# jianhao2016/AllSet

Measured on AMD Instinct MI355X. Metric: edges*d aggregated / sec (V->E->V layer fwd+bwd), higher is better.
Workload: dtype f32

## Files before the change

allset_amd/csrc/fused_fwd2.hip:

```cpp
#include <stdlib.h>

#include "common.h"
#include "mfma.h"

namespace allset {

constexpr int kF2Block = 768;
constexpr int kF2Rows = 32;
constexpr int kF2VWaves = 8;
constexpr int kF2Sets = 4;

#ifdef ALLSET_ABL5_NOBAR
#define ALLSET_TICK() ALLSET_TICK_NO_BARRIER()
#else
#define ALLSET_TICK() ALLSET_TICK_BARRIER()
#endif

template <bool HAS_LN, bool DROP_IN, bool DROP_OUT, bool D8, bool F16, int XM = 0, bool AUX = false>
__global__ __launch_bounds__(kF2Block) void fused_linear_fwd_roles_kernel(
    const float* __restrict__ x, int64_t ldx, const float* __restrict__ gamma, const float* __restrict__ beta, float eps,
    int relu_in, float p_in, uint64_t seed_in, const float* __restrict__ W, const float* __restrict__ bias, int relu_out,
    float p_out, uint64_t seed_out, float* __restrict__ y, int64_t ldy, float* __restrict__ stats, int64_t n,
    const uint64_t* __restrict__ seed_base, uint32_t* __restrict__ mask_out, int64_t xcb, int64_t ycb, float ln_inv,
    const float* __restrict__ colb = nullptr, float* __restrict__ uo = nullptr, int64_t lduo = 0,
// ... 139 lines not shown
        const float s = row16_sum(((t[0].x + t[0].y) + (t[0].z + t[0].w)) + ((t[1].x + t[1].y) + (t[1].z + t[1].w)));
        const float mean = s * inv_k;
        float q2 = 0.f;
#pragma unroll
        for (int hb = 0; hb < 2; ++hb) {
          t[hb].x -= mean; t[hb].y -= mean; t[hb].z -= mean; t[hb].w -= mean;
          q2 = fmaf(t[hb].x, t[hb].x, fmaf(t[hb].y, t[hb].y, fmaf(t[hb].z, t[hb].z, fmaf(t[hb].w, t[hb].w, q2))));
        }
        const float rstd = rsqrtf(row16_sum(q2) * inv_k + eps);
        if (live && c == 0) *reinterpret_cast<float2*>(stats + (stage * R + lr) * 2) = make_float2(mean, rstd);
#pragma unroll
        for (int hb = 0; hb < 2; ++hb) {
          t[hb].x = fmaf(t[hb].x * rstd, gam[hb].x, bet[hb].x); t[hb].y = fmaf(t[hb].y * rstd, gam[hb].y, bet[hb].y);
          t[hb].z = fmaf(t[hb].z * rstd, gam[hb].z, bet[hb].z); t[hb].w = fmaf(t[hb].w * rstd, gam[hb].w, bet[hb].w);
        }
      }
      if constexpr (XM == 1) {
        if (live) {
          char* ub = reinterpret_cast<char*>(uo + stage * R * lduo) + static_cast<uint32_t>(lr) * static_cast<uint32_t>(lduo) * 4u + 16u * c;
          *reinterpret_cast<float4*>(ub) = t[0];
          *reinterpret_cast<float4*>(ub + 256) = t[1];
        }
      }
      if constexpr (AUX) {
        float s4[4];
#pragma unroll
        for (int j = 0; j < 4; ++j) {
          const float4 w0 = *reinterpret_cast<const float4*>(&sAuxW[j * KD + 4 * c]), w1 = *reinterpret_cast<const float4*>(&sAuxW[j * KD + 64 + 4 * c]);
          s4[j] = row16_sum(fmaf(t[0].x, w0.x, fmaf(t[0].y, w0.y, fmaf(t[0].z, w0.z, t[0].w * w0.w))) +
                              fmaf(t[1].x, w1.x, fmaf(t[1].y, w1.y, fmaf(t[1].z, w1.z, t[1].w * w1.w))));
        }
        if (live && c == 0)
          *reinterpret_cast<float4*>(aux_out + (stage * R + lr) * 4) =
              make_float4(s4[0] + sAuxW[4 * KD], s4[1] + sAuxW[4 * KD + 1], s4[2] + sAuxW[4 * KD + 2], s4[3] + sAuxW[4 * KD + 3]);
      }
      float rsc = su1;
      if constexpr (ROWSC) {
        float amax = 0.f;
#pragma unroll
        for (int hb = 0; hb < 2; ++hb)
          amax = fmaxf(fmaxf(fmaxf(fabsf(t[hb].x), fabsf(t[hb].y)), fmaxf(fabsf(t[hb].z), fabsf(t[hb].w))), amax);
        amax = fmaxf(amax, dpp_row<0xB1>(amax)); amax = fmaxf(amax, dpp_row<0x4E>(amax));
        amax = fmaxf(amax, dpp_row<0x141>(amax)); amax = fmaxf(amax, dpp_row<0x140>(amax));
        const int e = min(max(static_cast<int>(__float_as_uint(amax * keep_in) >> 23), 20), 254);
        eC = eB; eB = eA; eA = e;
        rsc = __uint_as_float(static_cast<uint32_t>(254 + 13 - e) << 23);
      }
#pragma unroll
      for (int hb = 0; hb < 2; ++hb) {
        if constexpr (DROP_IN) {
          const float4 kp = keep4(seed_in, stage, hb, thr_in, keep_in);
          t[hb].x *= kp.x; t[hb].y *= kp.y; t[hb].z *= kp.z; t[hb].w *= kp.w;
        }
        if constexpr (ROWSC || XM == 1) { t[hb].x *= rsc; t[hb].y *= rsc; t[hb].z *= rsc; t[hb].w *= rsc; }
        const int wo = swizzle256(lr, 128 * hb + 8 * c);
        if constexpr (F16) {
          uint32_t h0, l0, h1, l1;
          split2_f16(t[hb].x, t[hb].y, h0, l0);
          split2_f16(t[hb].z, t[hb].w, h1, l1);
          *reinterpret_cast<uint2*>(img + 0 * PLANE + wo) = make_uint2(h0, h1);
          *reinterpret_cast<uint2*>(img + 1 * PLANE + wo) = make_uint2(l0, l1);
        } else {
          uint32_t h0, m0, l0, h1, m1, l1;
          split3_bf16(t[hb].x, t[hb].y, h0, m0, l0);
          split3_bf16(t[hb].z, t[hb].w, h1, m1, l1);
          *reinterpret_cast<uint2*>(img + 0 * PLANE + wo) = make_uint2(h0, h1);
          *reinterpret_cast<uint2*>(img + 1 * PLANE + wo) = make_uint2(m0, m1);
          *reinterpret_cast<uint2*>(img + 2 * PLANE + wo) = make_uint2(l0, l1);
        }
      }
      __builtin_amdgcn_sched_barrier(0);
      request_x(k + kF2Sets, xr);
      __builtin_amdgcn_sched_barrier(0);
    };
    auto E = [&](int64_t k, int erow) {
      const int64_t stage = stage_of(k);
      const int nrows = rows_left(stage);
      const bool live = lr < nrows;
      const float* ty = sY + (k & 1) * (R * SPY);
      char* yb = reinterpret_cast<char*>(y + stage * R * ldy);
      const uint32_t yo = static_cast<uint32_t>(lr) * static_cast<uint32_t>(ldy) * 4u + coy0;
      const float unsc = ROWSC ? __uint_as_float(static_cast<uint32_t>(erow - 13) << 23) : 1.f;
      float4 vv[2];
#pragma unroll
      for (int hb = 0; hb < 2; ++hb) {
        float4 v = *reinterpret_cast<const float4*>(&ty[lr * SPY + 64 * hb + 4 * c]);
        if constexpr (ROWSC) {
          v.x = fmaf(v.x, unsc, bia[hb].x); v.y = fmaf(v.y, unsc, bia[hb].y); v.z = fmaf(v.z, unsc, bia[hb].z); v.w = fmaf(v.w, unsc, bia[hb].w);
        } else {
          v.x += bia[hb].x; v.y += bia[hb].y; v.z += bia[hb].z; v.w += bia[hb].w;
        }
        if (relu_out) { v.x = fmaxf(v.x, 0.f); v.y = fmaxf(v.y, 0.f); v.z = fmaxf(v.z, 0.f); v.w = fmaxf(v.w, 0.f); }
        vv[hb] = v;
      }
      if constexpr (XM == 2) {
        float4 sv[2];
        float a1 = 0.f;
#pragma unroll
        for (int hb = 0; hb < 2; ++hb) {
          sv[hb] = make_float4(resR[hb].x + vv[hb].x, resR[hb].y + vv[hb].y, resR[hb].z + vv[hb].z, resR[hb].w + vv[hb].w);
          a1 += (sv[hb].x + sv[hb].y) + (sv[hb].z + sv[hb].w);
        }
        const float mean = row16_sum(a1) * (1.f / 128.f);
        float q2 = 0.f;
        float4 cv[2];
#pragma unroll
        for (int hb = 0; hb < 2; ++hb) {
          cv[hb] = make_float4(sv[hb].x - mean, sv[hb].y - mean, sv[hb].z - mean, sv[hb].w - mean);
          q2 = fmaf(cv[hb].x, cv[hb].x, fmaf(cv[hb].y, cv[hb].y, fmaf(cv[hb].z, cv[hb].z, fmaf(cv[hb].w, cv[hb].w, q2))));
        }
        const float rstd = rsqrtf(row16_sum(q2) * (1.f / 128.f) + eps);
        if (live) {
          if (c == 0) *reinterpret_cast<float2*>(stats + (stage * R + lr) * 2) = make_float2(mean, rstd);
          char* ub = reinterpret_cast<char*>(uo + stage * R * lduo) + static_cast<uint32_t>(lr) * static_cast<uint32_t>(lduo) * 4u + 16u * c;
          *reinterpret_cast<float4*>(ub) = sv[0];
          *reinterpret_cast<float4*>(ub + 256) = sv[1];
        }
#pragma unroll
        for (int hb = 0; hb < 2; ++hb) {
          float4 o = make_float4(fmaf(cv[hb].x * rstd, gam[hb].x, bet[hb].x), fmaf(cv[hb].y * rstd, gam[hb].y, bet[hb].y),
                                 fmaf(cv[hb].z * rstd, gam[hb].z, bet[hb].z), fmaf(cv[hb].w * rstd, gam[hb].w, bet[hb].w));
          if (relu_post) { o.x = fmaxf(o.x, 0.f); o.y = fmaxf(o.y, 0.f); o.z = fmaxf(o.z, 0.f); o.w = fmaxf(o.w, 0.f); }
          if constexpr (DROP_OUT) {
            const float4 kp = keep4(seed_out, stage, hb, thr_out, keep_out);
            o.x *= kp.x; o.y *= kp.y; o.z *= kp.z; o.w *= kp.w;
          }
          if (live) *reinterpret_cast<float4*>(yb + hb * dhy + yo) = o;
        }
      }
#pragma unroll
      for (int hb = 0; hb < 2; ++hb) {
        float4 v = vv[hb];
        if constexpr (DROP_OUT && XM != 2) {
          const float4 kp = keep4(seed_out, stage, hb, thr_out, keep_out);
          v.x *= kp.x; v.y *= kp.y; v.z *= kp.z; v.w *= kp.w;
        }
        if constexpr (XM == 3 || XM == 4) vv[hb] = v;
#ifdef ALLSET_ABL5_NOSTORE
        if (live && v.x == 123.456f)
#else
        if (live && XM != 2 && XM != 3 && XM != 4)
#endif
          *reinterpret_cast<float4*>(yb + hb * dhy + yo) = v;
        if (mask_out != nullptr) {
          const uint64_t b0 = __ballot(v.x > 0.f), b1 = __ballot(v.y > 0.f), b2 = __ballot(v.z > 0.f), b3 = __ballot(v.w > 0.f);
          const int sh = 8 * (lane0 & 7);
          const uint32_t word = static_cast<uint32_t>((b0 >> sh) & 0xffu) | (static_cast<uint32_t>((b1 >> sh) & 0xffu) << 8) |
                                (static_cast<uint32_t>((b2 >> sh) & 0xffu) << 16) | (static_cast<uint32_t>((b3 >> sh) & 0xffu) << 24);
          if (lane0 < 8 && 16 * (wave >> 2) < nrows)
            mask_out[((stage * (R / 16) + (wave >> 2)) * (ND / 64) + hb) * 32 + (wave & 3) * 8 + lane0] = word;
        }
      }
      if constexpr (XM == 3 || XM == 4) {
        uint32_t u[2][4], own[2], oth[2];
        const uint32_t sh = 4u * (c & 7);
#pragma unroll
        for (int hb = 0; hb < 2; ++hb) {
          u[hb][0] = __float_as_uint(vv[hb].x); u[hb][1] = __float_as_uint(vv[hb].y);
          u[hb][2] = __float_as_uint(vv[hb].z); u[hb][3] = __float_as_uint(vv[hb].w);
          const uint32_t nib = (u[hb][0] != 0u ? 1u : 0u) | (u[hb][1] != 0u ? 2u : 0u) | (u[hb][2] != 0u ? 4u : 0u) | (u[hb][3] != 0u ? 8u : 0u);
          float mw = __uint_as_float(nib << sh);
          mw = __uint_as_float(__float_as_uint(mw) | __float_as_uint(dpp_row<0xB1>(mw)));
          mw = __uint_as_float(__float_as_uint(mw) | __float_as_uint(dpp_row<0x4E>(mw)));
          mw = __uint_as_float(__float_as_uint(mw) | __float_as_uint(dpp_row<0x141>(mw)));
          own[hb] = __float_as_uint(mw);
          oth[hb] = __float_as_uint(dpp_row<0x140>(mw));
        }
        const bool hi = c >= 8;
        const uint32_t below = (1u << sh) - 1u;
        const int cnt0 = __popc(own[0]) + __popc(oth[0]);
        const int kocc = cnt0 + __popc(own[1]) + __popc(oth[1]);
        int pos[2];
        pos[0] = 4 + (hi ? __popc(oth[0]) : 0) + __popc(own[0] & below);
        pos[1] = 4 + cnt0 + (hi ? __popc(oth[1]) : 0) + __popc(own[1] & below);
        uint32_t* im = reinterpret_cast<uint32_t*>(sY + (k & 1) * (R * SPY) + lr * SPY);
        __builtin_amdgcn_fence(__ATOMIC_SEQ_CST, "wavefront");
        __builtin_amdgcn_wave_barrier();
        if constexpr (XM == 4) {
          *reinterpret_cast<uint4*>(im + 4 * c) = make_uint4(0u, 0u, 0u, (128u + c) * 0x010101u | (static_cast<uint32_t>(kocc) << 24));
          uint8_t* imb = reinterpret_cast<uint8_t*>(im);
#pragma unroll
          for (int hb = 0; hb < 2; ++hb) {
            int j = pos[hb] - 4;
#pragma unroll
            for (int i = 0; i < 4; ++i) {
              const bool put = u[hb][i] != 0u && j < kCellCap;
              const int cl = 16 * (j & 15), sl = j >> 4;
              *reinterpret_cast<uint32_t*>(imb + (put ? cl + 4 * sl : 4 * (SPY - 1))) = u[hb][i];
              imb[put ? cl + 12 + sl : 4 * (SPY - 1)] = static_cast<uint8_t>(64 * hb + 4 * c + i);
              j += u[hb][i] != 0u ? 1 : 0;
            }
          }
        } else {
        *reinterpret_cast<uint4*>(im + 4 * c) = make_uint4(0u, 0u, 0u, 0u);
        *reinterpret_cast<uint4*>(im + (hi ? SPY - 4 : 0)) = make_uint4(own[0], oth[0], own[1], oth[1]);
#pragma unroll
        for (int hb = 0; hb < 2; ++hb)
#pragma unroll
          for (int i = 0; i < 4; ++i) {
            const bool occ = u[hb][i] != 0u;
            im[occ ? pos[hb] : SPY - 1] = u[hb][i];
            pos[hb] += occ ? 1 : 0;
          }
        }
        __builtin_amdgcn_fence(__ATOMIC_SEQ_CST, "wavefront");
        __builtin_amdgcn_wave_barrier();
        const uint4 o = *reinterpret_cast<const uint4*>(im + 4 * c);
        if (live) *reinterpret_cast<uint4*>(reinterpret_cast<uint32_t*>(uo) + (stage * R + lr) * kPackPitchDw + 4 * c) = o;
        if (live && kocc > (XM == 4 ? kCellCap : kPackCap)) {
          *reinterpret_cast<float4*>(yb + yo) = vv[0];
          *reinterpret_cast<float4*>(yb + 256 + yo) = vv[1];
        }
      }
      if constexpr (XM == 2) {
        __builtin_amdgcn_sched_barrier(0);
        request_res(k + 1);
        __builtin_amdgcn_sched_barrier(0);
      }
    };

    static_assert(kF2Sets == 4, "the trip below is written for four register sets");
#pragma unroll
    for (int q = 0; q < kF2Sets; ++q) request_x(q, xrS[q]);
    request_res(0);
    S0(0, xrS[0]);
    ALLSET_TICK();
    S0(1, xrS[1]);
    ALLSET_TICK();
#define ALLSET_F2_FULL_TICK(tt, set) do { ALLSET_MARK(3); S0((tt) + 1, xrS[set]); ALLSET_MARK(0); E((tt) - 1, eC); ALLSET_MARK(1); ALLSET_TICK(); ALLSET_MARK(2); } while (0)
    int64_t t = 1;
    for (; t + 3 < T; t += 4) {
      ALLSET_F2_FULL_TICK(t, 2);
      ALLSET_F2_FULL_TICK(t + 1, 3);
      ALLSET_F2_FULL_TICK(t + 2, 0);
      ALLSET_F2_FULL_TICK(t + 3, 1);
    }
    if (t < T) ALLSET_F2_FULL_TICK(t, 2);
    if (t + 1 < T) ALLSET_F2_FULL_TICK(t + 1, 3);
    if (t + 2 < T) ALLSET_F2_FULL_TICK(t + 2, 0);
#undef ALLSET_F2_FULL_TICK
    E(T - 1, eB);
  } else {
    const int m = wave - kF2VWaves;
    Frag wq[2][4][F16 ? 2 : 3];
    float inv_s = 1.f;
    if constexpr (F16) {
      const int nn = lane0 & 15, kg = lane0 >> 4;
      float4 wa[2][4], wb[2][4];
      float amax = 0.f;
#pragma unroll
      for (int ct = 0; ct < 2; ++ct)
#pragma unroll
        for (int tt = 0; tt < 4; ++tt) {
          const float4* wr = reinterpret_cast<const float4*>(W + (32 * m + 16 * ct + nn) * KD + 32 * kg + 8 * tt);
          wa[ct][tt] = wr[0]; wb[ct][tt] = wr[1];
          amax = fmaxf(fmaxf(fmaxf(fabsf(wa[ct][tt].x), fabsf(wa[ct][tt].y)), fmaxf(fabsf(wa[ct][tt].z), fabsf(wa[ct][tt].w))), amax);
          amax = fmaxf(fmaxf(fmaxf(fabsf(wb[ct][tt].x), fabsf(wb[ct][tt].y)), fmaxf(fabsf(wb[ct][tt].z), fabsf(wb[ct][tt].w))), amax);
        }
#pragma unroll
      for (int off = 1; off < 64; off <<= 1) amax = fmaxf(amax, __shfl_xor(amax, off));
      const int ew = __builtin_amdgcn_readfirstlane(min(max(static_cast<int>(__float_as_uint(amax) >> 23), 20), 254));
      const float sw = __uint_as_float(static_cast<uint32_t>(254 + 13 - ew) << 23);
      const int X = ew - 140 - Su, X1 = X >> 1, X2 = X - X1;
      inv_s = __uint_as_float(static_cast<uint32_t>(127 + X1) << 23) * __uint_as_float(static_cast<uint32_t>(127 + X2) << 23);
#pragma unroll
      for (int ct = 0; ct < 2; ++ct)
#pragma unroll
        for (int tt = 0; tt < 4; ++tt) {
          const float4 a = wa[ct][tt], b = wb[ct][tt];
          uint32_t ph[4], pl[4];
          split2_f16(a.x * sw, a.y * sw, ph[0], pl[0]);
          split2_f16(a.z * sw, a.w * sw, ph[1], pl[1]);
          split2_f16(b.x * sw, b.y * sw, ph[2], pl[2]);
          split2_f16(b.z * sw, b.w * sw, ph[3], pl[3]);
          wq[ct][tt][0].u = make_uint4(ph[0], ph[1], ph[2], ph[3]);
          wq[ct][tt][1].u = make_uint4(pl[0], pl[1], pl[2], pl[3]);
        }
    } else {
      const int nn = lane0 & 15, kg = lane0 >> 4;
#pragma unroll
      for (int ct = 0; ct < 2; ++ct)
#pragma unroll
        for (int tt = 0; tt < 4; ++tt) {
          const float4* wr = reinterpret_cast<const float4*>(W + (32 * m + 16 * ct + nn) * KD + 32 * kg + 8 * tt);
          const float4 a = wr[0], b = wr[1];
          uint32_t ph[4], pm[4], pl[4];
          split3_bf16(a.x, a.y, ph[0], pm[0], pl[0]);
          split3_bf16(a.z, a.w, ph[1], pm[1], pl[1]);
          split3_bf16(b.x, b.y, ph[2], pm[2], pl[2]);
          split3_bf16(b.z, b.w, ph[3], pm[3], pl[3]);
          wq[ct][tt][0].u = make_uint4(ph[0], ph[1], ph[2], ph[3]);
          wq[ct][tt][1].u = make_uint4(pm[0], pm[1], pm[2], pm[3]);
          wq[ct][tt][2].u = make_uint4(pl[0], pl[1], pl[2], pl[3]);
        }
    }
    auto S1 = [&](int64_t k) {
      ALLSET_FRESH_LANE(lane);
      const int ri = lane & 15, kg = lane >> 4;
      const uint8_t* img = sX + (k & 1) * IMG;
      float* ty = sY + (k & 1) * (R * SPY);
      constexpr int NP = F16 ? 2 : 3;
      auto load_a = [&](Frag (&f0)[3], Frag (&f1)[3], int tt) {
        const int o0 = swizzle256(ri, 64 * kg + 16 * tt), o1 = swizzle256(16 + ri, 64 * kg + 16 * tt);
#pragma unroll
        for (int pl = 0; pl < NP; ++pl) {
          f0[pl].u = *reinterpret_cast<const uint4*>(img + pl * PLANE + o0);
          f1[pl].u = *reinterpret_cast<const uint4*>(img + pl * PLANE + o1);
        }
      };
      Frag fa0[2][3], fa1[2][3];
      f32x4 acc[2][2];
#pragma unroll
      for (int a = 0; a < 2; ++a)
#pragma unroll
        for (int b = 0; b < 2; ++b) acc[a][b] = f32x4{0.f, 0.f, 0.f, 0.f};
      load_a(fa0[0], fa1[0], 0);
#pragma unroll
      for (int tt = 0; tt < 4; ++tt) {
        if (tt + 1 < 4) load_a(fa0[(tt + 1) & 1], fa1[(tt + 1) & 1], tt + 1);
        const Frag (&a0)[3] = fa0[tt & 1];
        const Frag (&a1)[3] = fa1[tt & 1];
        constexpr int PA_[6] = {2, 0, 1, 1, 0, 0}, PB_[6] = {0, 2, 1, 0, 1, 0};
#ifdef ALLSET_ABL5_NOMFMA
        acc[0][0][0] += __builtin_bit_cast(float, a0[0].u.x ^ a0[1].u.y ^ a0[2].u.z); acc[1][0][0] += __builtin_bit_cast(float, a1[0].u.x ^ a1[1].u.y ^ a1[2].u.z);
        for (int pr = 0; pr < 0; ++pr) {
#else
#pragma unroll
        for (int pr = 0; pr < (F16 ? 0 : 6); ++pr) {
#endif
          if constexpr (!F16) {
            acc[0][0] = __builtin_amdgcn_mfma_f32_16x16x32_bf16(a0[PA_[pr]].v, wq[0][tt][PB_[pr]].v, acc[0][0], 0, 0, 0);
            acc[1][0] = __builtin_amdgcn_mfma_f32_16x16x32_bf16(a1[PA_[pr]].v, wq[0][tt][PB_[pr]].v, acc[1][0], 0, 0, 0);
            acc[0][1] = __builtin_amdgcn_mfma_f32_16x16x32_bf16(a0[PA_[pr]].v, wq[1][tt][PB_[pr]].v, acc[0][1], 0, 0, 0);
            acc[1][1] = __builtin_amdgcn_mfma_f32_16x16x32_bf16(a1[PA_[pr]].v, wq[1][tt][PB_[pr]].v, acc[1][1], 0, 0, 0);
          }
        }
#ifndef ALLSET_ABL5_NOMFMA
        if constexpr (F16) {
          constexpr int QA_[3] = {1, 0, 0}, QB_[3] = {0, 1, 0};
#pragma unroll
          for (int pr = 0; pr < 3; ++pr) {
            acc[0][0] = __builtin_amdgcn_mfma_f32_16x16x32_f16(a0[QA_[pr]].h, wq[0][tt][QB_[pr]].h, acc[0][0], 0, 0, 0);
            acc[1][0] = __builtin_amdgcn_mfma_f32_16x16x32_f16(a1[QA_[pr]].h, wq[0][tt][QB_[pr]].h, acc[1][0], 0, 0, 0);
            acc[0][1] = __builtin_amdgcn_mfma_f32_16x16x32_f16(a0[QA_[pr]].h, wq[1][tt][QB_[pr]].h, acc[0][1], 0, 0, 0);
            acc[1][1] = __builtin_amdgcn_mfma_f32_16x16x32_f16(a1[QA_[pr]].h, wq[1][tt][QB_[pr]].h, acc[1][1], 0, 0, 0);
          }
        }
#endif
        __builtin_amdgcn_sched_barrier(0);
      }
#pragma unroll
      for (int rt = 0; rt < 2; ++rt)
#pragma unroll
        for (int ct = 0; ct < 2; ++ct)
#pragma unroll
          for (int r = 0; r < 4; ++r) ty[(16 * rt + 4 * kg + r) * SPY + 32 * m + 16 * ct + ri] = F16 ? acc[rt][ct][r] * inv_s : acc[rt][ct][r];
    };
    ALLSET_TICK();
    for (int64_t k = 0; k < T; ++k) {
      ALLSET_MARK(3);
// ... 221 lines not shown
```

allset_amd/dense.py:

```python
from __future__ import annotations

import contextlib
import os
from ctypes import byref, c_int64
from typing import Optional, Tuple

import torch
from torch.autograd.function import once_differentiable

from . import _lib, _memo
from ._lib import check, ptr, require_device, stream_of, on_device
from .ops import _ld, _rowmajor, _timed

Tensor = torch.Tensor


class _SeedSource:
    base: Optional[Tensor] = None
    salt: int = 0


_SEED_SCRATCH = torch.empty((), dtype=torch.int64)


# ... 918 lines not shown
        _check_f32(x)
        x = x.contiguous()
        y = torch.empty_like(x)
        seed, base = _seed_for(p)
        n = x.numel()
        with on_device(dev), _timed("relu_dropout_fwd", dev, 2 * n * 4):
            check(_lib.load().allset_relu_dropout_fwd(ptr(x), p, seed, ptr(y), n, ptr(base),
                                                      stream_of(dev)), "allset_relu_dropout_fwd")
        ctx.save_for_backward(y)
        ctx.p = float(p)
        return y

    @staticmethod
    @once_differentiable
    def backward(ctx, gy):
        (y,) = ctx.saved_tensors
        dev = y.device
        gy = gy.contiguous()
        gx = torch.empty_like(y)
        n = y.numel()
        with on_device(dev), _timed("relu_dropout_bwd", dev, 3 * n * 4):
            check(_lib.load().allset_relu_dropout_bwd(ptr(gy), ptr(y), ctx.p, ptr(gx), n, stream_of(dev)),
                  "allset_relu_dropout_bwd")
        return gx, None


class _Linear(torch.autograd.Function):

    @staticmethod
    def forward(ctx, x, weight, bias):
        ctx.save_for_backward(x, weight)
        ctx.has_bias = bias is not None
        ctx.params = (weight, bias)
        return torch.nn.functional.linear(x, weight, bias)

    @staticmethod
    @once_differentiable
    def backward(ctx, gy):
        x, weight = ctx.saved_tensors
        gy = gy.contiguous()
        gx = gw = gb = None
        need_w, need_b = ctx.needs_input_grad[1], ctx.has_bias and ctx.needs_input_grad[2]
        if need_w and linear_narrow_supported(gy, x, weight):
            defer = ctx.params if (not ctx.has_bias or need_b) else None
            gx, gw, gb = linear_narrow_bwd(gy, x, weight, ctx.needs_input_grad[0], defer_to=defer)
            return gx, gw, gb if need_b else None
        if ctx.needs_input_grad[0]:
            gx = gy @ weight
        if need_w or need_b:
            if wgrad_supported(gy, x):
                gw, gb = wgrad(gy, x, want_bias=need_b)
            elif (gy.is_cuda and gy.dtype == x.dtype and gy.dtype in (torch.float32, torch.bfloat16) and x.dim() == 2
                  and gy.shape[0] >= 8192):
                gw, gb = wgrad_padded(gy, x, want_bias=need_b)
            else:
                gw = gy.t() @ x
                gb = gy.sum(dim=0) if need_b else None
        return gx, gw, gb


class _FusedNormLinear(torch.autograd.Function):

    @staticmethod
    def forward(ctx, x, gamma, beta, weight, bias, eps, relu_in, p_in, relu_out, p_out, in_cb=0, out_cb=0):
        seed_in = _draw_seed() if p_in > 0.0 else 0
        seed_out = _draw_seed() if p_out > 0.0 else 0
        base = _seed_base() if (p_in > 0.0 or p_out > 0.0) else None
        keep_y = relu_out or p_out > 0.0
        words = activation_mask_words(x.shape[0], weight.shape[0]) if (keep_y and any(ctx.needs_input_grad)) else 0
        mask = torch.empty(words, dtype=torch.int32, device=x.device) if words > 0 else None
        if in_cb or out_cb:
            n_rows = x.shape[0] // (weight.shape[1] // in_cb) if in_cb else x.shape[0]
            words = activation_mask_words(n_rows, weight.shape[0]) if (keep_y and any(ctx.needs_input_grad)) else 0
            mask = torch.empty(words, dtype=torch.int32, device=x.device) if words > 0 else None
            y, stats = fused_linear_fwd_blocked(x, in_cb, weight, bias, gamma, beta, eps, relu_in, p_in, seed_in, relu_out, p_out,
                                                seed_out, base, mask, out_cb)
        else:
            y, stats = fused_linear_fwd(x, weight, bias, gamma, beta, eps, relu_in, p_in, seed_in, relu_out, p_out, seed_out,
                                        base, mask)
        ctx.save_for_backward(x, stats, gamma, beta, weight, y if (keep_y and mask is None) else None, mask)
        ctx.cfg = (bool(relu_in), float(p_in), seed_in, float(p_out), bias is not None, base)
        ctx.layout = (int(in_cb), int(out_cb))
        ctx.params = (gamma, beta, weight, bias)
        return y

    @staticmethod
    @once_differentiable
    def backward(ctx, gy):
        x, stats, gamma, beta, weight, y, mask = ctx.saved_tensors
        relu_in, p_in, seed_in, p_out, has_bias, base = ctx.cfg
        if x.shape[0] == 0:
            z = lambda t, need: torch.zeros_like(t) if (t is not None and need) else None
            return (z(x, ctx.needs_input_grad[0]), z(gamma, ctx.needs_input_grad[1]), z(beta, ctx.needs_input_grad[2]),
                    z(weight, ctx.needs_input_grad[3]),
                    weight.new_zeros(weight.shape[0]) if (has_bias and ctx.needs_input_grad[4]) else None,
                    None, None, None, None, None, None, None)
        gy = gy.contiguous()
        gx = dg = db = gw = gb = None
        need_b = has_bias and ctx.needs_input_grad[4]
        in_cb, out_cb = ctx.layout
        if in_cb or out_cb:
            gx, dg, db, gw, gb = fused_linear_bwd_all_blocked(gy, out_cb, mask, p_out, weight, x, in_cb, stats, gamma, beta, relu_in,
                                                              p_in, seed_in, base, want_bias=need_b)
            return gx, dg, db, gw, gb, None, None, None, None, None, None, None
        if (ctx.needs_input_grad[0] and ctx.needs_input_grad[3] and y is None and x.shape[0] > 0 and
                (gamma is not None or one_pass_preferred(weight.shape[0], weight.shape[1])) and
                fused_linear_bwd_all_supported(weight.shape[0], weight.shape[1], gamma is not None, p_in > 0.0, relu_in,
                                               mask is not None)):
            need = ctx.needs_input_grad
            defer = ctx.params if (_Deferred.active and (gamma is None or (need[1] and need[2])) and (not has_bias or need[4])) else None
            gx, dg, db, gw, gb = fused_linear_bwd_all(gy, mask, p_out, weight, x, stats, gamma, beta, relu_in, p_in, seed_in,
                                                      base, want_bias=need_b, defer_to=defer)
            return gx, dg, db, gw, gb, None, None, None, None, None, None, None
        if ctx.needs_input_grad[3] or need_b:
            gw, gb = wgrad_fused(gy, y, p_out, x, stats, gamma, beta, relu_in, p_in, seed_in, want_bias=need_b,
                                 seed_base=base, mask=mask)
        if ctx.needs_input_grad[0] or (gamma is not None and (ctx.needs_input_grad[1] or ctx.needs_input_grad[2])):
            gx, dg, db = fused_linear_bwd(gy, y, p_out, weight, x, stats, gamma, relu_in, p_in, seed_in, base, mask,
                                          want_gx=ctx.needs_input_grad[0])
        return gx, dg, db, gw, gb, None, None, None, None, None, None, None


class PackedRows:

    __slots__ = ("packed", "_side", "format")

    def __init__(self, packed: Tensor, side: Tensor, format: str):
        from . import ops
        ops.packed_format_entry(format, "PackedRows")
        self.packed, self._side, self.format = packed, side, format

    @property
    def shape(self):
        return self._side.shape


class _FusedNormLinearPacked(torch.autograd.Function):

    @staticmethod
    def forward(ctx, x, gamma, beta, weight, bias, eps, relu_in, p_in, relu_out, p_out, fmt):
        from . import ops
        seed_in = _draw_seed()
        seed_out = _draw_seed()
        base = _seed_base()
        words = activation_mask_words(x.shape[0], weight.shape[0]) if any(ctx.needs_input_grad) else 0
        mask = torch.empty(words, dtype=torch.int32, device=x.device) if words > 0 else None
        packed, side, stats = ops.fused_linear_fwd_packed(x, weight, bias, gamma, beta, eps, relu_in, p_in, seed_in, relu_out, p_out, seed_out,
                                                          base, mask, _arith_for(0, weight.shape[1], weight.shape[0], True, 0), fmt=fmt)
        ctx.save_for_backward(x, stats, gamma, beta, weight, None, mask)
        ctx.cfg = (bool(relu_in), float(p_in), seed_in, float(p_out), bias is not None, base)
        ctx.layout = (0, 0)
        ctx.params = (gamma, beta, weight, bias)
        ctx.mark_non_differentiable(packed)
        return side, packed

    @staticmethod
    @once_differentiable
    def backward(ctx, gy, _g_packed=None):
        return _FusedNormLinear.backward(ctx, gy)[:10] + (None,)


def fused_norm_linear_packed_supported(x: Tensor, gamma: Optional[Tensor], weight: Tensor, p_in: float, relu_out: bool, p_out: float,
                                       format: str) -> bool:
    from . import ops
    N, K = weight.shape
    return (x.is_cuda and x.dtype == torch.float32 and x.dim() == 2 and x.shape[0] > 0 and gamma is not None and bool(relu_out)
            and ops.fused_linear_fwd_packed_supported(K, N, True, p_in, p_out, fmt=format))


def fused_norm_linear_packed(x: Tensor, gamma: Tensor, beta: Tensor, weight: Tensor, bias: Optional[Tensor], eps: float, relu_in: bool,
                             p_in: float, relu_out: bool, p_out: float, format: str) -> PackedRows:
    if not fused_norm_linear_packed_supported(x, gamma, weight, p_in, relu_out, p_out, format):
        raise _lib.AllSetHipError("fused_norm_linear_packed: built for a [128, 128] Linear behind a LayerNorm with relu_out and both "
                                  "dropouts active only (fused_norm_linear_packed_supported)")
    side, packed = _FusedNormLinearPacked.apply(x, gamma, beta, weight, bias, float(eps), bool(relu_in), float(p_in), bool(relu_out),
                                                float(p_out), format)
    return PackedRows(packed, side, format)


class _WideNormLinear(torch.autograd.Function):

    @staticmethod
    def forward(ctx, x, gamma, beta, weight, bias, eps, relu_in, p_in, relu_out, p_out, stats_in=None, emit=None):
        seed_in = _draw_seed() if p_in > 0.0 else 0
        seed_out = _draw_seed() if p_out > 0.0 else 0
        base = _seed_base() if (p_in > 0.0 or p_out > 0.0) else None
        stats = (stats_in if stats_in is not None else row_stats(x, relu_in, eps)) if gamma is not None else None
        stats_y = torch.empty((x.shape[0], 2), dtype=torch.float32, device=x.device) if emit is not None else None
        keep_y = relu_out or p_out > 0.0
        words = activation_mask_words(x.shape[0], weight.shape[0]) if (keep_y and x.shape[0] > 0) else 0
        mask = torch.empty(words, dtype=torch.int32, device=x.device) if words > 0 else None
        f16 = wide_f16(gamma is not None)
        planes, ctx.planes_t = (prefetched_planes(weight, False), prefetched_planes(weight, True)) if f16 else (None, None)
        y = gemm_x6(x, planes or gemm_x6_planes(weight, False, f16=f16), weight.shape[0], bias, relu_in=relu_in, stats=stats, gamma=gamma,
                    beta=beta, p_in=p_in, seed_in=seed_in, relu_out=relu_out, p_out=p_out, seed_out=seed_out, seed_base=base,
                    mask_out=mask, stats_out=stats_y, stats_eps=emit[0] if emit is not None else 1e-5,
                    stats_relu=bool(emit[1]) if emit is not None else False)
        ctx.save_for_backward(x, stats, gamma, beta, weight, y if (keep_y and mask is None) else None, mask)
        ctx.cfg = (bool(relu_in), float(p_in), seed_in, float(p_out), bias is not None, base)
        ctx.params = (gamma, beta, weight, bias)
        if emit is None:
            return y
        ctx.mark_non_differentiable(stats_y)
        return y, stats_y

    @staticmethod
    @once_differentiable
    def backward(ctx, gy, _g_stats=None):
        x, stats, gamma, beta, weight, y, mask = ctx.saved_tensors
        relu_in, p_in, seed_in, p_out, has_bias, base = ctx.cfg
        if x.shape[0] == 0:
            z = lambda t, need: torch.zeros_like(t) if (t is not None and need) else None
            return (z(x, ctx.needs_input_grad[0]), z(gamma, ctx.needs_input_grad[1]), z(beta, ctx.needs_input_grad[2]),
                    z(weight, ctx.needs_input_grad[3]),
                    weight.new_zeros(weight.shape[0]) if (has_bias and ctx.needs_input_grad[4]) else None,
                    None, None, None, None, None, None, None)
        gy = gy.contiguous()
        gx = dg = db = gw = gb = None
        need_b = has_bias and ctx.needs_input_grad[4]
        need = ctx.needs_input_grad
        p_g, p_bt, p_w, p_b = ctx.params
        dfr = _Deferred.active
        if ctx.needs_input_grad[3] or need_b:
            gw, gb = wgrad_fused(gy, y, p_out, x, stats, gamma, beta, relu_in, p_in, seed_in, want_bias=need_b, seed_base=base, mask=mask,
                                 defer_to=(p_w, p_b) if (dfr and need[3] and (not has_bias or need[4])) else None)
        need_x = ctx.needs_input_grad[0]
        if need_x or (gamma is not None and (ctx.needs_input_grad[1] or ctx.needs_input_grad[2])):
            planes_t = ctx.planes_t if (ctx.planes_t is not None and wide_f16()) else gemm_x6_planes(weight, True)
            if gamma is not None and weight.shape[1] <= 256:
                gx, dg, db = gemm_x6_lnb(gy, planes_t, x, stats, gamma, relu_in, p_in, seed_in, mask_y=y,
                                         p_mask=p_out, seed_base=base, mask_bits=mask,
                                         defer_to=(p_g, p_bt) if (dfr and need[1] and need[2]) else None)
                return gx, dg, db, gw, gb, None, None, None, None, None, None, None
            sgn = x if (gamma is None and relu_in and planes_t.f16 and x.stride(-1) == 1 and x.stride(0) % 4 == 0 and x.data_ptr() % 16 == 0
                        and _lib.load().allset_gemm_wide_sgn_supported(_lib.ARITH_FP16X3, weight.shape[1], weight.shape[0])) else None
            gu = gemm_x6(gy, planes_t, weight.shape[1], None, mask_y=y, p_mask=p_out, mask_bits=mask, sgn_x=sgn)
            if gamma is not None:
                gx, dg, db = ln_bwd(gu, x, stats, gamma, relu_in, p_in, seed_in, base, want_gx=need_x,
                                    defer_to=(p_g, p_bt) if (dfr and need[1] and need[2]) else None)
            elif relu_in and sgn is None:
                gx = torch.empty_like(x)
                with torch.cuda.device(x.device), _timed("relu_dropout_bwd", x.device, 3 * x.numel() * 4):
                    check(_lib.load().allset_relu_dropout_bwd(ptr(gu), ptr(x.contiguous()), 0.0, ptr(gx), x.numel(),
                                                              stream_of(x.device)), "allset_relu_dropout_bwd")
            else:
                gx = gu
        return gx, dg, db, gw, gb, None, None, None, None, None, None, None


def wide_linear_supported(K: int, N: int, has_ln: bool, relu_in: bool = False, p_in: float = 0.0) -> bool:
    if fused_linear_supported(K, N) or not x6_active() or not gemm_x6_supported(N, K) or not gemm_x6_supported(K, N):
        return False
    if has_ln:
        return K <= 512 and K % 4 == 0
    return p_in == 0.0


def wide_stats_chain_supported(K: int, N: int, has_ln: bool, relu_in: bool = False, p_in: float = 0.0) -> bool:
    return N == 256 and wide_linear_supported(K, N, has_ln, relu_in, p_in)


def fused_norm_linear(x: Tensor, gamma: Optional[Tensor], beta: Optional[Tensor], weight: Tensor, bias: Optional[Tensor],
                      eps: float = 1e-5, relu_in: bool = False, p_in: float = 0.0, relu_out: bool = False,
                      p_out: float = 0.0, in_cb: int = 0, out_cb: int = 0, stats_in: Optional[Tensor] = None,
                      emit_stats: Optional[Tuple[float, bool]] = None):
    if p_out > 0.0 and not relu_out:
        raise _lib.AllSetHipError("fused_norm_linear: an output dropout needs relu_out=True")
    N, K = weight.shape
    if in_cb or out_cb:
        if not blocked_linear_supported(K, N):
            raise _lib.AllSetHipError(f"fused_norm_linear: column-blocked operands are not built for a [{N}, {K}] weight")
        return _FusedNormLinear.apply(x, gamma, beta, weight, bias, float(eps), bool(relu_in), float(p_in), bool(relu_out),
                                      float(p_out), int(in_cb), int(out_cb))
    if fused_linear_supported(K, N):
        if stats_in is not None or emit_stats is not None:
            raise _lib.AllSetHipError("fused_norm_linear: stats_in / emit_stats belong to the tiled wide path")
        return _FusedNormLinear.apply(x, gamma, beta, weight, bias, float(eps), bool(relu_in), float(p_in), bool(relu_out), float(p_out))
    if emit_stats is not None and N != 256:
        raise _lib.AllSetHipError("fused_norm_linear: emit_stats needs 256 output features")
    if stats_in is None and emit_stats is None:
        return _WideNormLinear.apply(x, gamma, beta, weight, bias, float(eps), bool(relu_in), float(p_in), bool(relu_out), float(p_out))
    return _WideNormLinear.apply(x, gamma, beta, weight, bias, float(eps), bool(relu_in), float(p_in), bool(relu_out), float(p_out),
                                 stats_in, (float(emit_stats[0]), bool(emit_stats[1])) if emit_stats is not None else None)


def ln_res_supported(d: int, dtype: torch.dtype = torch.float32) -> bool:
    if dtype == torch.bfloat16:
        return bool(_lib.load().allset_ln_bf16_supported(d))
    return dtype == torch.float32 and bool(_lib.load().allset_ln_res_supported(d))


def ln_res_fwd(x: Tensor, colb: Optional[Tensor], res: Optional[Tensor], gamma: Tensor, beta: Tensor, eps: float,
               relu_out: bool, p: float, seed: int, seed_base: Optional[Tensor] = None) -> Tuple[Tensor, Tensor]:
    dev = require_device(x, colb, res, gamma, beta)
    bf16 = x.dtype == torch.bfloat16
    if bf16:
        _check_dtype(torch.bfloat16, x, colb, res, gamma, beta)
    else:
        _check_f32(x, colb, res, gamma, beta)
    x = _rowmajor(x)
    res = _rowmajor(res) if res is not None else None
    n, d = x.shape
    y = torch.empty((n, d), dtype=x.dtype, device=dev)
    stats = torch.empty((n, 2), dtype=torch.float32, device=dev)
    lib = _lib.load()
    fn, name = (lib.allset_ln_res_fwd_bf16, "allset_ln_res_fwd_bf16") if bf16 else (lib.allset_ln_res_fwd, "allset_ln_res_fwd")
    with on_device(dev), _timed("ln_res_fwd", dev, (2 + (res is not None)) * n * d * x.element_size()):
        check(fn(ptr(x), _ld(x), ptr(colb.contiguous() if colb is not None else None), ptr(res), _ld(res) if res is not None else 0,
                 ptr(gamma.contiguous()), ptr(beta.contiguous()), eps, int(relu_out), p, seed, ptr(y), max(d, 1), ptr(stats), n, d,
                 ptr(seed_base), stream_of(dev)), name)
    return y, stats


def ln_res_bwd(gy: Tensor, x: Tensor, colb: Optional[Tensor], res: Optional[Tensor], stats: Tensor, gamma: Tensor,
               beta: Tensor, relu_out: bool, p: float, seed: int, seed_base: Optional[Tensor] = None, defer_to=None
               ) -> Tuple[Tensor, Tensor, Tensor, Tensor]:
    dev = require_device(gy, x, colb, res, stats, gamma, beta)
    bf16 = x.dtype == torch.bfloat16
    if bf16:
        _check_dtype(torch.bfloat16, gy, x, colb, res, gamma, beta)
    gy, x = _rowmajor(gy), _rowmajor(x)
    res = _rowmajor(res) if res is not None else None
    n, d = x.shape
    lib = _lib.load()
    npart = c_int64(0)
    if bf16:
        check(lib.allset_ln_bwd_bf16_partials(n, d, byref(npart)), "allset_ln_bwd_bf16_partials")
    else:
        check(lib.allset_ln_res_bwd_partials(n, d, byref(npart)), "allset_ln_res_bwd_partials")
    partials = torch.empty((npart.value, 3, d), dtype=torch.float32, device=dev)
    gs = torch.empty((n, d), dtype=x.dtype, device=dev)
    fn, name = (lib.allset_ln_res_bwd_bf16, "allset_ln_res_bwd_bf16") if bf16 else (lib.allset_ln_res_bwd, "allset_ln_res_bwd")
    with on_device(dev), _timed("ln_res_bwd", dev, (3 + (res is not None)) * n * d * x.element_size()):
        check(fn(ptr(gy), _ld(gy), ptr(x), _ld(x), ptr(colb.contiguous() if colb is not None else None), ptr(res),
                 _ld(res) if res is not None else 0, ptr(stats), ptr(gamma.contiguous()), ptr(beta.contiguous()), int(relu_out), p,
                 seed, ptr(gs), max(d, 1), ptr(partials), npart.value, n, d, ptr(seed_base), stream_of(dev)), name)
    if not bf16 and defer_to is not None:
        dg_, db_, dc_ = _defer_or_reduce(partials, [(defer_to[0], 0, (d,)), (defer_to[1], d, (d,)),
                                                    (defer_to[2] if colb is not None else None, 2 * d,
                                                     tuple(defer_to[2].shape) if (colb is not None and defer_to[2] is not None) else (d,))], True)
        return gs, dg_, db_, dc_
    if bf16 and (3 * d) % 4 == 0 and npart.value <= 4096:
        red = reduce_partials_to(partials.view(npart.value, 3 * d), 3 * d, torch.bfloat16).view(3, d)
    else:
        red = reduce_partials(partials)
        if bf16:
            red = red.to(torch.bfloat16)
    return gs, red[0], red[1], red[2]


def ln_res_bwd_pma_supported(d: int, heads: int, dtype: torch.dtype = torch.float32) -> bool:
    if dtype == torch.bfloat16:
        return bool(_lib.load().allset_ln_res_bwd_pma_bf16_supported(d, heads))
    return dtype == torch.float32 and bool(_lib.load().allset_ln_res_bwd_pma_supported(d, heads))


def ln_res_bwd_pma(gy: Tensor, x: Tensor, colb: Tensor, stats: Tensor, gamma: Tensor, beta: Tensor, m: Tensor, l: Tensor,
                   defer_to=None) -> Tuple[Tensor, Tensor, Tensor, Tensor, Tensor]:
    dev = require_device(gy, x, colb, stats, gamma, beta, m, l)
    bf16 = x.dtype == torch.bfloat16
    if bf16:
# ... 933 lines not shown
    if x.shape[1] >= 256 and not replaceable and _lib.load().allset_sparse_ln_linear_supported(weight.shape[0]):
        sp = sparse_rows(x)
        if sp is not None:
            return _SparseInputNormLinear.apply(x, sp, gamma, beta, weight, bias, float(eps), float(p_pre))
    return _InputNormLinear.apply(x, gamma, beta, weight, bias, float(eps), float(p_pre))


import contextlib
import threading

_sync_bn_state = threading.local()


@contextlib.contextmanager
def sync_bn_rows(valid_rows: int, group=None):
    prev = getattr(_sync_bn_state, "scope", None)
    _sync_bn_state.scope = (int(valid_rows), group)
    try:
        yield
    finally:
        _sync_bn_state.scope = prev


def _host_all_reduce_sum(t: Tensor, group) -> Tensor:
    import torch.distributed as dist
    if not (dist.is_available() and dist.is_initialized()) or dist.get_world_size(group) == 1:
        return t
    if t.is_cuda and dist.get_backend(group) == "gloo":
        h = t.cpu()
        dist.all_reduce(h, group=group)
        return h.to(t.device)
    dist.all_reduce(t, group=group)
    return t


class _SyncBatchNorm(torch.autograd.Function):
    @staticmethod
    def forward(ctx, x, weight, bias, valid, group, eps):
        xs = x[:valid].float()
        d = x.shape[1]
        head = torch.cat([xs.sum(0), xs.new_full((1,), float(valid))])
        head = _host_all_reduce_sum(head, group)
        count = head[d].clamp(min=1.0)
        mean = head[:d] / count
        m2 = _host_all_reduce_sum(((xs - mean) ** 2).sum(0), group)
        var = m2 / count
        rstd = torch.rsqrt(var + eps)
        xhat = (x.float() - mean) * rstd
        y = xhat * weight.float() + bias.float() if weight is not None else xhat
        ctx.save_for_backward(xhat, weight, rstd, count)
        ctx.cfg = (int(valid), group, bias is not None)
        ctx.mark_non_differentiable(mean, var, count)
        return y.to(x.dtype), mean, var, count

    @staticmethod
    @once_differentiable
    def backward(ctx, gy, _gm, _gv, _gc):
        xhat, weight, rstd, count = ctx.saved_tensors
        valid, group, has_bias = ctx.cfg
        g = gy.float()
        gs, xs = g[:valid], xhat[:valid]
        loc = torch.cat([gs.sum(0), (gs * xs).sum(0)])
        d = g.shape[1]
        glob = _host_all_reduce_sum(loc.clone(), group)
        w = weight.float() if weight is not None else torch.ones_like(rstd)
        gx = torch.zeros_like(g)
        gx[:valid] = (gs - glob[:d] / count - xs * (glob[d:] / count)) * (w * rstd)
        if valid < g.shape[0]:
            gx[valid:] = g[valid:] * (w * rstd)
        gw = loc[d:].to(weight.dtype) if weight is not None else None
        gb = loc[:d].to(weight.dtype) if (weight is not None and has_bias) else None
        return gx.to(gy.dtype), gw, gb, None, None, None



def col_moments_supported(d: int) -> bool:
    return bool(_lib.load().allset_col_moments_supported(int(d)))


def col_moments(x: Tensor, relu_in: bool = False, center: Optional[Tensor] = None) -> Tensor:
    dev = require_device(x, center)
    _check_f32(x, center)
    x = _rowmajor(x)
    n, d = x.shape
    lib = _lib.load()
    ns = c_int64(0)
    check(lib.allset_col_moments_slices(n, byref(ns)), "allset_col_moments_slices")
    part = torch.empty((ns.value, d), dtype=torch.float32, device=dev)
    with on_device(dev), _timed("col_moments", dev, n * d * 4):
        check(lib.allset_col_moments(ptr(x), _ld(x), n, d, int(relu_in), ptr(center.contiguous() if center is not None else None),
                                     ptr(part), ns.value, stream_of(dev)), "allset_col_moments")
    return reduce_partials(part) if ns.value > 1 else part[0]


def col_mean_var(x: Tensor, relu_in: bool = False) -> Tuple[Tensor, Tensor]:
    dev = require_device(x)
    _check_f32(x)
    x = _rowmajor(x)
    n, d = x.shape
    lib = _lib.load()
    ns = c_int64(0)
    check(lib.allset_col_moments_slices(n, byref(ns)), "allset_col_moments_slices")
    part = torch.empty((ns.value, 2, d), dtype=torch.float64, device=dev)
    with on_device(dev), _timed("col_moments", dev, n * d * 4):
        check(lib.allset_col_moments2(ptr(x), _ld(x), n, d, int(relu_in), ptr(part), ns.value, stream_of(dev)), "allset_col_moments2")
    tot = part.sum(0) if ns.value > 1 else part[0]
    mean = tot[0] / n
    var = (tot[1] / n - mean * mean).clamp_(min=0.0)
    return mean.float(), var.float()


def col_affine_add_(gx: Tensor, x: Tensor, s: Tensor, t: Tensor, relu_mask: bool) -> Tensor:
    dev = require_device(gx, x, s, t)
    _check_f32(gx, x, s, t)
    n, d = x.shape
    with on_device(dev), _timed("col_affine_add", dev, 3 * n * d * 4):
        check(_lib.load().allset_col_affine_add(ptr(gx), _ld(gx), ptr(x), _ld(x), ptr(s.contiguous()), ptr(t.contiguous()),
                                                int(relu_mask), n, d, stream_of(dev)), "allset_col_affine_add")
    return gx


def bn_linear_supported(bn, lin, x: Optional[Tensor] = None) -> bool:
    ok = (bn.affine and bn.weight is not None and bn.weight.dtype == torch.float32 and lin.weight.dtype == torch.float32 and
          lin.bias is not None and lin.in_features == bn.num_features and
          fused_linear_supported(lin.in_features, lin.out_features) and
          bool(_lib.load().allset_fused_linear_bwd_all_supported(lin.out_features, lin.in_features, 1, 1, 1, 1, 0)) and
          col_moments_supported(lin.in_features))
    if ok and x is not None:
        ok = (x.is_cuda and x.dtype == torch.float32 and x.dim() == 2 and x.shape[0] >= 2 and x.shape[1] == lin.in_features and
              x.data_ptr() % 16 == 0 and x.stride(1) == 1 and x.stride(0) % 4 == 0)
    return ok


class _BatchNormLinear(torch.autograd.Function):

    @staticmethod
    def forward(ctx, x, bn_weight, bn_bias, weight, bias, eps, relu_in, p_in, relu_out, p_out):
        n, d = x.shape
        mean, var = col_mean_var(x, relu_in)
        rstd = torch.rsqrt(var + eps)
        a = bn_weight.float() * rstd
        b = bn_bias.float() - mean * a
        seed_in = _draw_seed() if p_in > 0.0 else 0
        seed_out = _draw_seed() if p_out > 0.0 else 0
        base = _seed_base() if (p_in > 0.0 or p_out > 0.0) else None
        keep_y = relu_out or p_out > 0.0
        words = activation_mask_words(n, weight.shape[0]) if (keep_y and any(ctx.needs_input_grad)) else 0
        mask = torch.empty(words, dtype=torch.int32, device=x.device) if words > 0 else None
        y, stats = fused_linear_fwd(x, weight, bias, a, b, 1.0, relu_in, p_in, seed_in, relu_out, p_out, seed_out, base, mask,
                                    norm_mode=1)
        ctx.save_for_backward(x, stats, a, b, weight, mask, mean, rstd, bn_weight)
        ctx.cfg = (bool(relu_in), float(p_in), seed_in, float(p_out), base, keep_y)
        ctx.mark_non_differentiable(mean, var)
        return y, mean, var

    @staticmethod
    @once_differentiable
    def backward(ctx, gy, _gm, _gv):
        x, stats, a, b, weight, mask, mean, rstd, bn_weight = ctx.saved_tensors
        relu_in, p_in, seed_in, p_out, base, keep_y = ctx.cfg
        if keep_y and mask is None:
            raise _lib.AllSetHipError("_BatchNormLinear: the forward ran without gradients enabled (no activation mask was kept)")
        n = x.shape[0]
        gx, g_a, g_b, gw, gb = fused_linear_bwd_all(gy.contiguous(), mask, p_out, weight, x, stats, a, b, relu_in, p_in, seed_in, base,
                                                    want_bias=True, norm_mode=1)
        core = g_a - mean * g_b
        dgamma = rstd * core
        dvar = -0.5 * rstd * rstd * rstd * bn_weight.float() * core
        dmean = -a * g_b
        s = dvar * (2.0 / n)
        t = dmean / n - s * mean
        if ctx.needs_input_grad[0]:
            col_affine_add_(gx, x, s, t, relu_in)
        else:
            gx = None
        return gx, dgamma.to(bn_weight.dtype), g_b.to(bn_weight.dtype), gw, gb, None, None, None, None, None


def bn_linear(bn, lin, x: Tensor, relu_in: bool, p_in: float, relu_out: bool = False, p_out: float = 0.0) -> Tensor:
    y, mean, var = _BatchNormLinear.apply(x, bn.weight, bn.bias, lin.weight, lin.bias, float(bn.eps), bool(relu_in), float(p_in),
                                          bool(relu_out), float(p_out))
    if bn.track_running_stats and bn.running_mean is not None:
        with torch.no_grad():
            n = x.shape[0]
            bn.num_batches_tracked += 1
            mom = bn.momentum if bn.momentum is not None else 1.0 / float(bn.num_batches_tracked)
            bn.running_mean.mul_(1.0 - mom).add_(mean.to(bn.running_mean.dtype), alpha=mom)
            bn.running_var.mul_(1.0 - mom).add_((var * (n / max(n - 1.0, 1.0))).to(bn.running_var.dtype), alpha=mom)
    return y


def batch_norm(bn: torch.nn.modules.batchnorm._BatchNorm, x: Tensor) -> Tensor:
    scope = getattr(_sync_bn_state, "scope", None)
    use_batch = bn.training or (bn.running_mean is None and bn.running_var is None)
    if scope is None or not use_batch:
        return bn(x)
    valid, group = scope
    valid = max(0, min(valid, x.shape[0]))
    y, mean, var, count = _SyncBatchNorm.apply(x, bn.weight, bn.bias, valid, group, float(bn.eps))
    if bn.training and bn.track_running_stats and bn.running_mean is not None:
        with torch.no_grad():
            bn.num_batches_tracked += 1
            mom = bn.momentum if bn.momentum is not None else 1.0 / float(bn.num_batches_tracked)
            unbiased = var * (count / (count - 1.0).clamp(min=1.0))
            bn.running_mean.mul_(1.0 - mom).add_(mean.to(bn.running_mean.dtype), alpha=mom)
            bn.running_var.mul_(1.0 - mom).add_(unbiased.to(bn.running_var.dtype), alpha=mom)
    return y
```

Measured before the change: 251.5 billion.

## Use DPP prefix-sum for packed cell positions and stage cell slots as dwords

```diff
diff --git a/allset_amd/csrc/fused_fwd2.hip b/allset_amd/csrc/fused_fwd2.hip
--- a/allset_amd/csrc/fused_fwd2.hip
+++ b/allset_amd/csrc/fused_fwd2.hip
@@ -315,43 +315,69 @@
         }
       }
       if constexpr (XM == 3 || XM == 4) {
-        uint32_t u[2][4], own[2], oth[2];
+        uint32_t u[2][4], own[2] = {0u, 0u}, oth[2] = {0u, 0u};
+        int pos[2], kocc;
         const uint32_t sh = 4u * (c & 7);
+        const bool hi = c >= 8;
 #pragma unroll
         for (int hb = 0; hb < 2; ++hb) {
           u[hb][0] = __float_as_uint(vv[hb].x); u[hb][1] = __float_as_uint(vv[hb].y);
           u[hb][2] = __float_as_uint(vv[hb].z); u[hb][3] = __float_as_uint(vv[hb].w);
-          const uint32_t nib = (u[hb][0] != 0u ? 1u : 0u) | (u[hb][1] != 0u ? 2u : 0u) | (u[hb][2] != 0u ? 4u : 0u) | (u[hb][3] != 0u ? 8u : 0u);
-          float mw = __uint_as_float(nib << sh);
-          mw = __uint_as_float(__float_as_uint(mw) | __float_as_uint(dpp_row<0xB1>(mw)));
-          mw = __uint_as_float(__float_as_uint(mw) | __float_as_uint(dpp_row<0x4E>(mw)));
-          mw = __uint_as_float(__float_as_uint(mw) | __float_as_uint(dpp_row<0x141>(mw)));
-          own[hb] = __float_as_uint(mw);
-          oth[hb] = __float_as_uint(dpp_row<0x140>(mw));
-        }
-        const bool hi = c >= 8;
-        const uint32_t below = (1u << sh) - 1u;
-        const int cnt0 = __popc(own[0]) + __popc(oth[0]);
-        const int kocc = cnt0 + __popc(own[1]) + __popc(oth[1]);
-        int pos[2];
-        pos[0] = 4 + (hi ? __popc(oth[0]) : 0) + __popc(own[0] & below);
-        pos[1] = 4 + cnt0 + (hi ? __popc(oth[1]) : 0) + __popc(own[1] & below);
+        }
+        if constexpr (XM == 4) {
+          int n2[2];
+#pragma unroll
+          for (int hb = 0; hb < 2; ++hb)
+            n2[hb] = ((u[hb][0] != 0u ? 1 : 0) + (u[hb][1] != 0u ? 1 : 0)) + ((u[hb][2] != 0u ? 1 : 0) + (u[hb][3] != 0u ? 1 : 0));
+          const int pk = n2[0] | (n2[1] << 8);
+          int inc = pk, tot = pk;
+          inc += __builtin_amdgcn_update_dpp(0, inc, 0x111, 0xf, 0xf, true);
+          inc += __builtin_amdgcn_update_dpp(0, inc, 0x112, 0xf, 0xf, true);
+          inc += __builtin_amdgcn_update_dpp(0, inc, 0x114, 0xf, 0xf, true);
+          inc += __builtin_amdgcn_update_dpp(0, inc, 0x118, 0xf, 0xf, true);
+          tot += __builtin_amdgcn_update_dpp(0, tot, 0xB1, 0xf, 0xf, false);
+          tot += __builtin_amdgcn_update_dpp(0, tot, 0x4E, 0xf, 0xf, false);
+          tot += __builtin_amdgcn_update_dpp(0, tot, 0x141, 0xf, 0xf, false);
+          tot += __builtin_amdgcn_update_dpp(0, tot, 0x140, 0xf, 0xf, false);
+          const int exc = inc - pk, cnt0 = tot & 0xff;
+          kocc = cnt0 + (tot >> 8);
+          pos[0] = 4 + (exc & 0xff);
+          pos[1] = 4 + cnt0 + (exc >> 8);
+        } else {
+#pragma unroll
+          for (int hb = 0; hb < 2; ++hb) {
+            const uint32_t nib = (u[hb][0] != 0u ? 1u : 0u) | (u[hb][1] != 0u ? 2u : 0u) | (u[hb][2] != 0u ? 4u : 0u) | (u[hb][3] != 0u ? 8u : 0u);
+            float mw = __uint_as_float(nib << sh);
+            mw = __uint_as_float(__float_as_uint(mw) | __float_as_uint(dpp_row<0xB1>(mw)));
+            mw = __uint_as_float(__float_as_uint(mw) | __float_as_uint(dpp_row<0x4E>(mw)));
+            mw = __uint_as_float(__float_as_uint(mw) | __float_as_uint(dpp_row<0x141>(mw)));
+            own[hb] = __float_as_uint(mw);
+            oth[hb] = __float_as_uint(dpp_row<0x140>(mw));
+          }
+          const uint32_t below = (1u << sh) - 1u;
+          const int cnt0 = __popc(own[0]) + __popc(oth[0]);
+          kocc = cnt0 + __popc(own[1]) + __popc(oth[1]);
+          pos[0] = 4 + (hi ? __popc(oth[0]) : 0) + __popc(own[0] & below);
+          pos[1] = 4 + cnt0 + (hi ? __popc(oth[1]) : 0) + __popc(own[1] & below);
+        }
         uint32_t* im = reinterpret_cast<uint32_t*>(sY + (k & 1) * (R * SPY) + lr * SPY);
         __builtin_amdgcn_fence(__ATOMIC_SEQ_CST, "wavefront");
         __builtin_amdgcn_wave_barrier();
         if constexpr (XM == 4) {
-          *reinterpret_cast<uint4*>(im + 4 * c) = make_uint4(0u, 0u, 0u, (128u + c) * 0x010101u | (static_cast<uint32_t>(kocc) << 24));
-          uint8_t* imb = reinterpret_cast<uint8_t*>(im);
+          static_assert(kCellCap == 48 && kCellCap + 3 < 64 && 64 + kCellCap + 3 < SPY, "three slots per cell; the staged columns sit 64 dwords above the values");
+          const uint32_t dcol = 128u + c;
+#pragma unroll
+          for (int s = 0; s < 3; ++s) { im[16 * s + c] = 0u; im[64 + 16 * s + c] = dcol; }
 #pragma unroll
           for (int hb = 0; hb < 2; ++hb) {
-            int j = pos[hb] - 4;
+            int j = min(pos[hb] - 4, kCellCap);
 #pragma unroll
             for (int i = 0; i < 4; ++i) {
-              const bool put = u[hb][i] != 0u && j < kCellCap;
-              const int cl = 16 * (j & 15), sl = j >> 4;
-              *reinterpret_cast<uint32_t*>(imb + (put ? cl + 4 * sl : 4 * (SPY - 1))) = u[hb][i];
-              imb[put ? cl + 12 + sl : 4 * (SPY - 1)] = static_cast<uint8_t>(64 * hb + 4 * c + i);
-              j += u[hb][i] != 0u ? 1 : 0;
+              const bool occ = u[hb][i] != 0u;
+              const int at = occ ? j : kCellCap;
+              im[at] = u[hb][i];
+              im[64 + at] = static_cast<uint32_t>(64 * hb + 4 * c + i);
+              j += occ ? 1 : 0;
             }
           }
         } else {
@@ -368,7 +394,11 @@
         }
         __builtin_amdgcn_fence(__ATOMIC_SEQ_CST, "wavefront");
         __builtin_amdgcn_wave_barrier();
-        const uint4 o = *reinterpret_cast<const uint4*>(im + 4 * c);
+        uint4 o;
+        if constexpr (XM == 4)
+          o = make_uint4(im[c], im[16 + c], im[32 + c], (im[64 + c] | (im[80 + c] << 8)) | ((im[96 + c] | (static_cast<uint32_t>(kocc) << 8)) << 16));
+        else
+          o = *reinterpret_cast<const uint4*>(im + 4 * c);
         if (live) *reinterpret_cast<uint4*>(reinterpret_cast<uint32_t*>(uo) + (stage * R + lr) * kPackPitchDw + 4 * c) = o;
         if (live && kocc > (XM == 4 ? kCellCap : kPackCap)) {
           *reinterpret_cast<float4*>(yb + yo) = vv[0];
diff --git a/allset_amd/dense.py b/allset_amd/dense.py
--- a/allset_amd/dense.py
+++ b/allset_amd/dense.py
@@ -1094,11 +1094,14 @@
         ctx.layout = (0, 0)
         ctx.params = (gamma, beta, weight, bias)
         ctx.mark_non_differentiable(packed)
+        ctx.set_materialize_grads(False)
         return side, packed
 
     @staticmethod
     @once_differentiable
     def backward(ctx, gy, _g_packed=None):
+        if gy is None:
+            return (None,) * 11
         return _FusedNormLinear.backward(ctx, gy)[:10] + (None,)
 
 
@@ -1144,11 +1147,14 @@
         if emit is None:
             return y
         ctx.mark_non_differentiable(stats_y)
+        ctx.set_materialize_grads(False)
         return y, stats_y
 
     @staticmethod
     @once_differentiable
     def backward(ctx, gy, _g_stats=None):
+        if gy is None:
+            return (None,) * 12
         x, stats, gamma, beta, weight, y, mask = ctx.saved_tensors
         relu_in, p_in, seed_in, p_out, has_bias, base = ctx.cfg
         if x.shape[0] == 0:
@@ -2388,11 +2394,14 @@
         ctx.save_for_backward(x, stats, a, b, weight, mask, mean, rstd, bn_weight)
         ctx.cfg = (bool(relu_in), float(p_in), seed_in, float(p_out), base, keep_y)
         ctx.mark_non_differentiable(mean, var)
+        ctx.set_materialize_grads(False)
         return y, mean, var
 
     @staticmethod
     @once_differentiable
-    def backward(ctx, gy, _gm, _gv):
+    def backward(ctx, gy, _gm=None, _gv=None):
+        if gy is None:
+            return (None,) * 10
         x, stats, a, b, weight, mask, mean, rstd, bn_weight = ctx.saved_tensors
         relu_in, p_in, seed_in, p_out, base, keep_y = ctx.cfg
         if keep_y and mask is None:
```

After: 254.6 billion (median of 6 runs). 1.2% higher.
